# i2Nav-WHU/IC-GVINS

Hardware: NVIDIA H100
Metric: frames/sec (KLT+BA) 1280x560 300-feat 10-KF window (higher is better)
Workload: dtype u8/int32 fixed point + f32 (KLT), f64 (BA)

## Files before the change

### ic_gvins_b200/csrc/ba.cu

```cuda
#include <cooperative_groups.h>
#include <unistd.h>
#include <math.h>
#include <stdlib.h>
#include <string.h>

#include <algorithm>
#include <string>
#include <thread>
#include <vector>

#include "ba_cull.cuh"
#include "ba_slide.cuh"
#include "preint.cuh"
#include "ba_math.cuh"
#include "common.cuh"
#include "geom_core.cuh"

namespace icg {
using namespace bam;
namespace cg = cooperative_groups;

constexpr int BA_SPLIT_W = 4;
constexpr int BA_CHOL_NB = 8;
constexpr int BA_MARG_MAXB = 72;
constexpr int BA_MAX_NODES = 32;

struct BaCaps {
    int NW, K, L, F, G, R;
    int NCV, N, NS, NCA, RJ, LP, NVB;
    int GQ;
};

struct WinDims {
    int K, L, F, n_imu, n_gnss, marg_r, marg_nb;
    int ext_const, td_const, reproj_huber, gnss_huber, has_imu_error, has_pose_prior, has_mix_prior;
    double reproj_sinv;
};

struct LmState {
    double radius, decrease_factor, x_cost, x_norm, cand_cost, model_cost_change, step_norm, gmax, initial_cost;
    double cost_cam[2];
    int iter, n_success, n_invalid, done, need_lin, last_success, first, step_valid, fresh_lin, max_iter, chol_ok;
    int lin_buf;
};

struct ShardDev {
    int split;
    int PK, BS, RV;
    double *peer[8];
    size_t off_inbox, off_bcast, off_scal, off_flagA, off_flagB, off_flagC;
    double *redv;
    int *err;
    double *slm;
    int *slm_cnt;
};

struct BaDev {
    ShardDev S;
    WinDims *dims;
    LmState *st;
    double *pose, *mix, *ext, *rho;
    double *pose_c, *mix_c, *ext_c, *rho_c;
    double *pose_0, *mix_0, *ext_0, *rho_0;
    uint8_t *f_active_0;
    double *gnss_std_0;
    uint8_t *f_active;
    int *lm_off;
    int *lm_perm;
    int *vb_lm0;
    int *ref_nrun;
    int *f_meta_s;
    double *f_const_s;
    int *vis_ord;
    int *part_off, *pair_ro, *npairs;
    double *gpart;
    int *vis_cnt;
    double *Mp[2];
    double *AW[2];
    double *costf[2];
    double *hl[2], *gl[2];
    double *Hc[2], *gc[2];
    double *scale_l, *scale_c;
    double *Hs;
    double *visv;
    double *imu_blob, *imu_U;
    int *gnss_node;
    double *gnss_blh, *gnss_std, *lever;
    double *pose_prior, *pose_prior_sinfo, *mix_prior, *mix_prior_std;
    int *marg_type, *marg_node;
    double *marg_x0, *marg_H0, *marg_b0, *marg_c0;
    double *cost_part;
    double *red2;
    int rank, world;
    double *step_c, *step_l;
    double *Sglobal;
    unsigned long long *clk;
};

__device__ __forceinline__ double *lin_Mp(const BaCaps &C, const BaDev &D, int b, int w) { return D.Mp[b] + (size_t) w * C.K * (C.K - 1) * 210; }
__device__ __forceinline__ double *lin_AW(const BaCaps &C, const BaDev &D, int b, int w) { return D.AW[b] + (size_t) w * C.LP * C.NCA; }
__device__ __forceinline__ double *lin_costf(const BaCaps &C, const BaDev &D, int b, int w) { return D.costf[b] + (size_t) w * C.F; }
__device__ __forceinline__ double *lin_hl(const BaCaps &C, const BaDev &D, int b, int w) { return D.hl[b] + (size_t) w * C.L; }
__device__ __forceinline__ double *lin_gl(const BaCaps &C, const BaDev &D, int b, int w) { return D.gl[b] + (size_t) w * C.L; }
__device__ __forceinline__ double *lin_Hc(const BaCaps &C, const BaDev &D, int b, int w) { return D.Hc[b] + (size_t) w * C.NS * C.NS; }
__device__ __forceinline__ double *lin_gc(const BaCaps &C, const BaDev &D, int b, int w) { return D.gc[b] + (size_t) w * C.NS; }

__device__ __forceinline__ int col_pose(int k) { return 6 * k; }
__device__ __forceinline__ int col_ext(int K) { return 6 * K; }
// ... 670 lines not shown
    __syncthreads();
    if (tid < 9 && dm.has_mix_prior) {
        const double sd = D.mix_prior_std[(size_t) w * 9 + tid];
        Hc[(size_t) (col_mix(K, 0) + tid) * C.NS + col_mix(K, 0) + tid] += 1.0 / (sd * sd);
        gc[col_mix(K, 0) + tid] += s_mp[tid] / sd;
    }
    __syncthreads();
    CAM_CLK(5)
#undef CAM_CLK
    return s_total;
}

constexpr int CAM_THREADS = 320;
__global__ void __launch_bounds__(CAM_THREADS) ba_lin_cam(BaCaps C, BaDev D, int at_cand) {
    extern __shared__ double smem[];
    const int w = blockIdx.x;
    LmState &st = D.st[w];
    if (st.done || !(at_cand ? st.step_valid : st.need_lin)) return;
    if (D.S.split && (w % D.world) != D.rank) return;
    const WinDims dm = D.dims[w];
    const int b = at_cand ? 1 - st.lin_buf : st.lin_buf;
    const double *pose = at_cand ? D.pose_c : D.pose, *mix = at_cand ? D.mix_c : D.mix, *ext = at_cand ? D.ext_c : D.ext;
    double c = cam_factors(C, D, w, dm, pose + (size_t) w * C.K * 7, mix + (size_t) w * C.K * 9, ext + (size_t) w * 8, true, b, smem);
    if (threadIdx.x == 0) st.cost_cam[b] = c;
}

constexpr int SOLVE_THREADS = 256;

__device__ __forceinline__ double block_sum(double v, double *s_red) {
    const int tid = threadIdx.x, lane = tid & 31, warp = tid >> 5;
    for (int o = 16; o > 0; o >>= 1) v += __shfl_down_sync(0xffffffffu, v, o);
    __syncthreads();
    if (lane == 0) s_red[warp] = v;
    __syncthreads();
    double t = 0;
    if (tid == 0) {
        for (int k = 0; k < (int) (blockDim.x >> 5); k++) t += s_red[k];
        s_red[32] = t;
    }
    __syncthreads();
    return s_red[32];
}
__device__ __forceinline__ double block_max(double v, double *s_red) {
    const int tid = threadIdx.x, lane = tid & 31, warp = tid >> 5;
    for (int o = 16; o > 0; o >>= 1) v = fmax(v, __shfl_down_sync(0xffffffffu, v, o));
    __syncthreads();
    if (lane == 0) s_red[warp] = v;
    __syncthreads();
    if (tid == 0) {
        double t = 0;
        for (int k = 0; k < (int) (blockDim.x >> 5); k++) t = fmax(t, s_red[k]);
        s_red[32] = t;
    }
    __syncthreads();
    return s_red[32];
}

__global__ void __launch_bounds__(SOLVE_THREADS, 2) ba_solve(BaCaps C, BaDev D) {
    extern __shared__ double sm[];
    const int w = blockIdx.x, tid = threadIdx.x;
    LmState &st = D.st[w];
    if (st.done) return;
#ifdef ICG_BA_PHASE_CLOCKS
    unsigned long long clk_prev = D.clk ? clock64() : 0ull;
#define SOLVE_CLK(k)                                              \
    if (D.clk && w == 0 && tid == 0) {                            \
        const unsigned long long t_ = clock64();                  \
        atomicAdd(&D.clk[k], t_ - clk_prev), atomicAdd(&D.clk[8 + (k)], 1ull); \
        clk_prev = t_;                                            \
    }
#define SOLVE_CLK_NOW() (D.clk ? clock64() : 0ull)
#define SOLVE_CLK_ADD(k, t0)                                      \
    if (D.clk && w == 0 && tid == 0) atomicAdd(&D.clk[k], clock64() - (t0)), atomicAdd(&D.clk[8 + (k)], 1ull);
#else
#define SOLVE_CLK(k)
#define SOLVE_CLK_NOW() 0ull
#define SOLVE_CLK_ADD(k, t0)
#endif
    const WinDims dm = D.dims[w];
    const int K = dm.K, L = dm.L, NCV = 6 * K + 7, N = 15 * K + 7;
    const int f_first = st.first, f_fresh = st.fresh_lin, f_last = st.last_success, f_iter = st.iter;
    const double f_gmax_old = st.gmax;
    (void) f_gmax_old;
    double *s_red = sm;
    double *s_scale = s_red + 40;
    double *s_g = s_scale + C.NS;
    double *s_rhs = s_g + C.NS;
    double *s_d2 = s_rhs + C.NS;
    double *s_diag = s_d2 + C.NS;
    double *S = s_diag + C.NS;
    const int b = st.lin_buf;
    const double *Hc = lin_Hc(C, D, b, w), *gcam = lin_gc(C, D, b, w), *Hs = D.Hs + (size_t) w * C.NS * C.NS;
    const double *V = D.visv + (size_t) (3 * C.NCV) * w;
    if (tid == 0 && st.need_lin) st.need_lin = 0;
    double *scale_c = D.scale_c + (size_t) w * C.NS;
    const double *hl = lin_hl(C, D, b, w), *gl = lin_gl(C, D, b, w), *scale_l = D.scale_l + (size_t) w * C.L;

    for (int a = tid; a < N; a += SOLVE_THREADS) {
        double g = gcam[a];
        if (a < NCV) g += V[NCV + a];
        s_g[a] = g;
        if (f_first) {
            double h = Hc[(size_t) a * C.NS + a] + (a < NCV ? V[a] : 0.0);
            scale_c[a] = 1.0 / (1.0 + sqrt(h));
        }
    }
    __syncthreads();
    for (int a = tid; a < N; a += SOLVE_THREADS) s_scale[a] = scale_c[a];
    double gmax_now = st.gmax;
    if (f_fresh) {
        double cs = 0, gq = 0;
        const double *costf = lin_costf(C, D, b, w);
        for (int f = tid; f < dm.F; f += SOLVE_THREADS) cs += costf[f];
        for (int l = tid; l < L; l += SOLVE_THREADS) gq = fmax(gq, fabs(gl[l]));
        const double c = block_sum(cs, s_red), gml = block_max(gq, s_red);
        double gm = 0;
        for (int a = tid; a < N; a += SOLVE_THREADS) gm = fmax(gm, fabs(s_g[a]));
        gm = fmax(block_max(gm, s_red), gml);
        gmax_now = gm;
        if (tid == 0) {
            st.x_cost = c + st.cost_cam[b];
            st.gmax = gm;
            if (f_first) st.initial_cost = st.x_cost;
            st.fresh_lin = 0;
        }
        __syncthreads();
    }
    if (f_first) {
        __syncthreads();
        if (tid == 0) st.first = 0;
    }
    {
        int term = 0;
        if (f_iter >= st.max_iter) term = 1;
        else if (f_last && gmax_now <= 1e-10) term = 2;
        else if (f_last && st.radius <= 1e-32) term = 2;
        if (term) {
            __syncthreads();
            if (tid == 0) st.done = term, st.step_valid = 0;
            return;
        }
    }
    __syncthreads();
    if (tid == 0) st.iter++;
    const double radius = st.radius;
    SOLVE_CLK(0)

    constexpr bool async_fill = true;
    if (async_fill) {
        for (int i = tid >> 5; i < N; i += SOLVE_THREADS / 32) {
            const double *src = (i < NCV ? Hs : Hc) + (size_t) i * C.NS;
            const unsigned dst = (unsigned) __cvta_generic_to_shared(S + i * (i + 1) / 2);
            for (int j = tid & 31; j <= i; j += 32)
                asm volatile("cp.async.ca.shared.global [%0], [%1], 8;" ::"r"(dst + 8u * j), "l"(src + j) : "memory");
        }
        asm volatile("cp.async.commit_group;" ::: "memory");
    }
    for (int a = tid; a < N; a += SOLVE_THREADS) {
        double h = Hc[(size_t) a * C.NS + a] + (a < NCV ? V[a] : 0.0);
        double hs = s_scale[a] * s_scale[a] * h;
        s_d2[a] = fmin(fmax(hs, 1e-6), 1e32) / radius;
        double gw = a < NCV ? V[2 * NCV + a] : 0.0;
        s_rhs[a] = -s_scale[a] * (s_g[a] - gw);
    }
    if (async_fill) asm volatile("cp.async.wait_all;" ::: "memory");
    __syncthreads();
    if (async_fill) {
        for (int i = tid >> 5; i < N; i += SOLVE_THREADS / 32) {
            double *row = S + i * (i + 1) / 2;
            const double si = s_scale[i];
            for (int j = tid & 31; j <= i; j += 32) {
                double v = si * s_scale[j] * row[j];
                if (i == j) v += s_d2[i];
                row[j] = v;
            }
        }
    } else {
        for (int i = tid >> 5; i < N; i += SOLVE_THREADS / 32) {
            constexpr int MAXQ = 16;
            double hv[MAXQ];
            const int nq = i / 32 + 1;
#pragma unroll
            for (int q = 0; q < MAXQ; q++) {
                const int j = (tid & 31) + 32 * q;
                hv[q] = 0;
                if (q < nq && j <= i) hv[q] = (i < NCV ? Hs : Hc)[(size_t) i * C.NS + j];
            }
#pragma unroll
            for (int q = 0; q < MAXQ; q++) {
                const int j = (tid & 31) + 32 * q;
                if (q < nq && j <= i) {
                    double v = s_scale[i] * s_scale[j] * hv[q];
                    if (i == j) v += s_d2[i];
                    S[i * (i + 1) / 2 + j] = v;
                }
            }
        }
    }
    for (int a = tid; a < N; a += SOLVE_THREADS) S[N * (N + 1) / 2 + a] = s_rhs[a];
    __syncthreads();
    SOLVE_CLK(1)
    __shared__ int s_fail;
    if (tid == 0) s_fail = 0;
    __syncthreads();
    const int NR = N + 1;
    for (int J0 = 0; J0 < N; J0 += BA_CHOL_NB) {
        const int nb = min(BA_CHOL_NB, N - J0);
        const int lane = tid & 31, warp = tid >> 5, g = lane >> 2, kk = lane & 3;
        const int ntile = (NR - J0 + 7) / 8;
        const unsigned long long pc0 = SOLVE_CLK_NOW();
        (void) pc0;
        const int cb = J0 + g;
        const double *rb = S + (cb < NR ? cb * (cb + 1) / 2 : 0);
        const bool okb = cb < NR;
        if (warp == 0) {
            if (J0 > 0) {
                const double *ra = rb;
                double acc[8] = {0, 0, 0, 0, 0, 0, 0, 0};
                int k0 = 0;
                for (; k0 + 16 <= J0; k0 += 16) {
                    const double x0 = okb ? ra[k0 + kk] : 0.0, x1 = okb ? ra[k0 + 4 + kk] : 0.0, x2 = okb ? ra[k0 + 8 + kk] : 0.0, x3 = okb ? ra[k0 + 12 + kk] : 0.0;
                    dmma884(acc[0], acc[1], x0, x0);
                    dmma884(acc[2], acc[3], x1, x1);
                    dmma884(acc[4], acc[5], x2, x2);
                    dmma884(acc[6], acc[7], x3, x3);
                }
                for (; k0 + 8 <= J0; k0 += 8) {
                    const double x0 = okb ? ra[k0 + kk] : 0.0, x1 = okb ? ra[k0 + 4 + kk] : 0.0;
                    dmma884(acc[0], acc[1], x0, x0);
                    dmma884(acc[2], acc[3], x1, x1);
                }
                const double c0 = (acc[0] + acc[2]) + (acc[4] + acc[6]), c1 = (acc[1] + acc[3]) + (acc[5] + acc[7]);
                const int i = J0 + g;
                if (i < NR) {
                    const int ca = J0 + 2 * kk;
                    if (ca < J0 + nb && ca <= i) S[i * (i + 1) / 2 + ca] -= c0;
                    if (ca + 1 < J0 + nb && ca + 1 <= i) S[i * (i + 1) / 2 + ca + 1] -= c1;
                }
                __syncwarp();
            }
            double Ld[BA_CHOL_NB][BA_CHOL_NB], dinv[BA_CHOL_NB];
            bool bad = false;
#pragma unroll
            for (int a = 0; a < BA_CHOL_NB; a++)
#pragma unroll
                for (int b = 0; b < BA_CHOL_NB; b++) Ld[a][b] = (a < nb && b <= a) ? S[(J0 + a) * (J0 + a + 1) / 2 + J0 + b] : (a == b ? 1.0 : 0.0);
#pragma unroll
            for (int j = 0; j < BA_CHOL_NB; j++) {
                double d = Ld[j][j];
#pragma unroll
                for (int k = 0; k < j; k++) d -= Ld[j][k] * Ld[j][k];
                if (!(d > 0.0) || !isfinite(d)) bad = true;
                const double di = rsqrt(d);
                dinv[j] = di;
                Ld[j][j] = d * di;
#pragma unroll
                for (int a = j + 1; a < BA_CHOL_NB; a++) {
                    double sum = Ld[a][j];
#pragma unroll
                    for (int k = 0; k < j; k++) sum -= Ld[a][k] * Ld[j][k];
                    Ld[a][j] = sum * di;
                }
            }
            __syncwarp();
            if (bad && lane == 0) s_fail = 1;
#pragma unroll
            for (int a2 = 0; a2 < BA_CHOL_NB; a2++) {
                double *ri = S + (J0 + a2) * (J0 + a2 + 1) / 2 + J0;
#pragma unroll
                for (int b = 0; b <= a2; b++)
                    if (lane == ((a2 * 8 + b) & 31) && a2 < nb) ri[b] = Ld[a2][b];
                if (lane == 8 + a2 && a2 < nb) s_diag[J0 + a2] = dinv[a2];
            }
            SOLVE_CLK_ADD(6, pc0)
        } else if (J0 > 0 && warp != 4) {
            constexpr int TPW = 4, NWARP = 6;
            const int wslot = warp < 4 ? warp - 1 : warp - 2;
            for (int t0 = 1 + wslot; t0 < ntile; t0 += TPW * NWARP) {
                const double *ra[TPW];
                bool oka[TPW];
                double acc[TPW][4];
#pragma unroll
                for (int u = 0; u < TPW; u++) {
                    const int ia = J0 + 8 * (t0 + u * NWARP) + g;
                    oka[u] = (t0 + u * NWARP) < ntile && ia < NR;
                    ra[u] = S + (oka[u] ? ia * (ia + 1) / 2 : 0);
                    acc[u][0] = acc[u][1] = acc[u][2] = acc[u][3] = 0;
                }
                for (int k0 = 0; k0 + 8 <= J0; k0 += 8) {
                    const double b0 = okb ? rb[k0 + kk] : 0.0, b1 = okb ? rb[k0 + 4 + kk] : 0.0;
                    double a0[TPW], a1[TPW];
#pragma unroll
                    for (int u = 0; u < TPW; u++) a0[u] = oka[u] ? ra[u][k0 + kk] : 0.0, a1[u] = oka[u] ? ra[u][k0 + 4 + kk] : 0.0;
#pragma unroll
                    for (int u = 0; u < TPW; u++) {
                        dmma884(acc[u][0], acc[u][1], a0[u], b0);
                        dmma884(acc[u][2], acc[u][3], a1[u], b1);
                    }
                }
#pragma unroll
                for (int u = 0; u < TPW; u++) {
                    const double c0 = acc[u][0] + acc[u][2], c1 = acc[u][1] + acc[u][3];
                    const int i = J0 + 8 * (t0 + u * NWARP) + g;
                    if (oka[u]) {
                        const int ca = J0 + 2 * kk;
                        if (ca < J0 + nb && ca <= i) S[i * (i + 1) / 2 + ca] -= c0;
                        if (ca + 1 < J0 + nb && ca + 1 <= i) S[i * (i + 1) / 2 + ca + 1] -= c1;
                    }
                }
            }
        }
        __syncthreads();
        const unsigned long long pc1 = SOLVE_CLK_NOW();
        (void) pc1;
        if (s_fail) break;
        for (int i = J0 + nb + tid; i < NR; i += SOLVE_THREADS) {
            double *ri = S + i * (i + 1) / 2 + J0;
            double x[BA_CHOL_NB];
#pragma unroll
            for (int c = 0; c < BA_CHOL_NB; c++) x[c] = c < nb ? ri[c] : 0.0;
#pragma unroll
            for (int c = 0; c < BA_CHOL_NB; c++) {
                if (c < nb) {
                    const double *lc = S + (J0 + c) * (J0 + c + 1) / 2 + J0;
                    double sum = x[c];
#pragma unroll
                    for (int k = 0; k < c; k++) sum -= x[k] * lc[k];
                    x[c] = sum * s_diag[J0 + c];
                }
            }
#pragma unroll
            for (int c = 0; c < BA_CHOL_NB; c++)
                if (c < nb) ri[c] = x[c];
        }
        __syncthreads();
        SOLVE_CLK_ADD(7, pc1)
    }
    __syncthreads();
    bool valid = !s_fail;
    SOLVE_CLK(2)
    if (valid) {
        double *y = S + N * (N + 1) / 2;
        const int lane = tid & 31;
        for (int J0 = ((N - 1) / BA_CHOL_NB) * BA_CHOL_NB; J0 >= 0; J0 -= BA_CHOL_NB) {
            const int nb = min(BA_CHOL_NB, N - J0);
            if (tid < 32) {
                double x[BA_CHOL_NB];
#pragma unroll
                for (int c = BA_CHOL_NB - 1; c >= 0; c--) {
                    x[c] = 0.0;
                    if (c < nb) {
                        double sum = y[J0 + c];
#pragma unroll
                        for (int k = BA_CHOL_NB - 1; k > c; k--)
                            if (k < nb) sum -= S[(J0 + k) * (J0 + k + 1) / 2 + J0 + c] * x[k];
                        x[c] = sum * s_diag[J0 + c];
                    }
                }
#pragma unroll
                for (int c = 0; c < BA_CHOL_NB; c++)
                    if (c == lane && c < nb) s_rhs[J0 + c] = x[c];
            }
            __syncthreads();
            for (int i = tid; i < J0; i += SOLVE_THREADS) {
                double acc = y[i];
#pragma unroll
                for (int c = BA_CHOL_NB - 1; c >= 0; c--)
                    if (c < nb) acc -= S[(J0 + c) * (J0 + c + 1) / 2 + i] * s_rhs[J0 + c];
                y[i] = acc;
            }
            __syncthreads();
        }
    }
    __syncthreads();
    SOLVE_CLK(3)
    double *step_l = D.step_l + (size_t) w * C.L;
    const double *AW = lin_AW(C, D, b, w);
    double part = 0;
    bool finite = true;
    double *R2 = D.red2 + (size_t) w * 4;
    if (!valid) {
        if (tid == 0) {
            st.chol_ok = 0, st.step_valid = 0;
            R2[0] = 0, R2[1] = 0, R2[2] = 1;
        }
        return;
    }
    for (int a = tid; a < N; a += SOLVE_THREADS) {
        double sp = s_rhs[a];
        finite = finite && isfinite(sp);
        part += -0.5 * sp * (s_scale[a] * s_g[a]) + 0.5 * s_d2[a] * sp * sp;
    }
    double *s_sx = s_diag;
    __syncthreads();
    for (int a = tid; a < NCV; a += SOLVE_THREADS) s_sx[a] = s_scale[a] * s_rhs[a];
    __syncthreads();
    {
        const int lane = tid & 31, warp = tid >> 5;
        constexpr int LB = 8;
        const int lu = ((lane >> 4) & 1) * 4 + ((lane >> 3) & 1) * 2 + ((lane >> 2) & 1);
        for (int l0 = LB * warp; l0 < L; l0 += LB * (SOLVE_THREADS / 32)) {
            const int l = l0 + lu;
            const bool lok = l < L;
            const double sl = lok ? scale_l[l] : 0.0, hh = lok ? hl[l] : 0.0, gg = lok ? gl[l] : 0.0;
            double d[LB];
#pragma unroll
            for (int u = 0; u < LB; u++) d[u] = 0;
            for (int c = lane; c < NCV; c += 32) {
                const double sx = s_sx[c];
#pragma unroll
                for (int u = 0; u < LB; u++) d[u] += (l0 + u < L ? AW[(size_t) (l0 + u) * C.NCA + c] : 0.0) * sx;
            }
            const double hs = sl * sl * hh, d2 = fmin(fmax(hs, 1e-6), 1e32) / radius, den = hs + d2, sg = sl * gg;
            double e4[4], e2[2];
            {
                const bool hi = lane & 16;
#pragma unroll
                for (int u = 0; u < 4; u++) {
                    const double keep = hi ? d[u + 4] : d[u], send = hi ? d[u] : d[u + 4];
                    e4[u] = keep + __shfl_xor_sync(0xffffffffu, send, 16);
                }
            }
            {
                const bool hi = lane & 8;
#pragma unroll
                for (int u = 0; u < 2; u++) {
                    const double keep = hi ? e4[u + 2] : e4[u], send = hi ? e4[u] : e4[u + 2];
                    e2[u] = keep + __shfl_xor_sync(0xffffffffu, send, 8);
                }
            }
            double mine;
            {
                const bool hi = lane & 4;
                const double keep = hi ? e2[1] : e2[0], send = hi ? e2[0] : e2[1];
                mine = keep + __shfl_xor_sync(0xffffffffu, send, 4);
            }
            mine += __shfl_xor_sync(0xffffffffu, mine, 2);
            mine += __shfl_xor_sync(0xffffffffu, mine, 1);
            if ((lane & 3) == 0 && lok) {
                double sp = (-sg - sl * mine) / den;
                finite = finite && isfinite(sp);
                step_l[l] = sp;
                part += -0.5 * sp * sg + 0.5 * d2 * sp * sp;
            }
        }
    }
    __syncthreads();
    SOLVE_CLK(4)
    const double mcc = block_sum(part, s_red);
    const double nfin = block_sum(finite ? 0.0 : 1.0, s_red);
    const double *pose = D.pose + (size_t) w * C.K * 7, *mix = D.mix + (size_t) w * C.K * 9, *ext = D.ext + (size_t) w * 8, *rho = D.rho + (size_t) w * C.L;
    double *pose_c = D.pose_c + (size_t) w * C.K * 7, *mix_c = D.mix_c + (size_t) w * C.K * 9, *ext_c = D.ext_c + (size_t) w * 8, *rho_c = D.rho_c + (size_t) w * C.L;
// ... 463 lines not shown
        return rc_init;
    }
    *out = h;
    return ICG_OK;
}

static int ba_create_body(icg_ba *h, int max_windows, int max_K, int max_L, int max_F, int max_gnss, int max_marg_r, void *stream) {
    if (stream) {
        h->stream = (cudaStream_t) stream;
    } else {
        ICG_CUDA(cudaStreamCreateWithFlags(&h->stream, cudaStreamNonBlocking));
        h->own_stream = true;
    }
    {
        int prio_lo = 0, prio_hi = 0;
        ICG_CUDA(cudaDeviceGetStreamPriorityRange(&prio_lo, &prio_hi));
        ICG_CUDA(cudaStreamCreateWithPriority(&h->stream_cam, cudaStreamNonBlocking, prio_hi));
    }
    ICG_CUDA(cudaEventCreateWithFlags(&h->ev_fork, cudaEventDisableTiming));
    ICG_CUDA(cudaEventCreateWithFlags(&h->ev_join, cudaEventDisableTiming));
    h->prof = getenv("ICG_BA_PROFILE") != nullptr;
    if (h->prof) {
        double *ck = nullptr;
        if (dmalloc(h, &ck, 48) != ICG_OK) return ICG_ENOMEM;
        h->D.clk = (unsigned long long *) ck;
    }
    if (getenv("ICG_BA_PROFILE_SKIP")) h->prof_skip = atoi(getenv("ICG_BA_PROFILE_SKIP"));
    BaCaps &C = h->C;
    max_L = std::max(1, max_L), max_F = std::max(1, max_F);
    C.NW = max_windows, C.K = max_K, C.L = max_L, C.F = max_F, C.G = std::max(1, max_gnss), C.R = std::max(1, max_marg_r);
    C.NCV = 6 * max_K + 7, C.N = 15 * max_K + 7, C.NS = (C.N + 3) & ~3, C.NCA = 4 * ((C.NCV + 1 + 3) / 4);
    C.RJ = (2 * max_F + 31) & ~31, C.LP = (max_L + 31) & ~31;
    C.NVB = (max_F + 127 - max_K) / (128 - max_K) + max_L / 128 + 4 + max_K;
    C.GQ = std::max(1, std::min(max_F, (C.NVB - 2) * (max_K - 1)));
    h->nblk_vis = (max_F + 255) / 256;
    const size_t NW = max_windows;
#define HD(field, count)                                                       \
    if (h->field.alloc(count) != ICG_OK) {                                     \
        set_error("icg_ba_create: allocation of " #field " failed");           \
        return ICG_ENOMEM;                                                     \
    }
    HD(dims, NW) HD(st, NW) HD(pose, NW * C.K * 7) HD(mix, NW * C.K * 9) HD(ext, NW * 8) HD(rho, NW * C.L)
    HD(imu_blob, NW * C.K * ICG_IMU_BLOB_DOUBLES) HD(imu_U, NW * C.K * 225) HD(gnss_blh, NW * C.G * 3) HD(gnss_std, NW * C.G * 3) HD(lever, NW * 3)
    HD(pose_prior, NW * 7) HD(pose_prior_sinfo, NW * 6) HD(mix_prior, NW * 9) HD(mix_prior_std, NW * 9) HD(marg_x0, NW * BA_MARG_MAXB * 9)
    HD(marg_H0, NW * C.R * C.R) HD(marg_b0, NW * C.R) HD(marg_c0, NW)
    HD(lm_off, NW * (C.L + 1)) HD(lm_perm, NW * C.L) HD(lm_fidx, NW * C.F) HD(gnss_node, NW * C.G) HD(marg_type, NW * BA_MARG_MAXB) HD(marg_node, NW * BA_MARG_MAXB) HD(f_active, NW * C.F)
    HD(scratch, 1024) HD(st_save, NW) HD(cull_counters, 2 * NW) HD(f_meta_s, NW * C.F * 4) HD(vb_lm0, NW * C.NVB) HD(ref_nrun, NW * C.K) HD(f_const_s, NW * C.F * 14)
    HD(part_off, NW * ((size_t) C.K * (C.K - 1) + 1)) HD(pair_ro, NW * (size_t) C.K * (C.K - 1)) HD(vis_ord, NW * C.F) HD(npairs, NW)
#undef HD
    ICG_CUDA(cudaMemsetAsync(h->st.d, 0, sizeof(LmState) * NW, h->stream));
    BaDev &D = h->D;
    D.rank = 0, D.world = 1;
    D.dims = h->dims.d, D.st = h->st.d, D.pose = h->pose.d, D.mix = h->mix.d, D.ext = h->ext.d, D.rho = h->rho.d;
    D.f_active = h->f_active.d;
    D.part_off = h->part_off.d, D.pair_ro = h->pair_ro.d, D.vis_ord = h->vis_ord.d, D.npairs = h->npairs.d;
    D.f_meta_s = h->f_meta_s.d, D.vb_lm0 = h->vb_lm0.d, D.ref_nrun = h->ref_nrun.d, D.f_const_s = h->f_const_s.d;
    D.lm_off = h->lm_off.d, D.lm_perm = h->lm_perm.d, D.imu_blob = h->imu_blob.d, D.imu_U = h->imu_U.d;
    D.gnss_node = h->gnss_node.d, D.gnss_blh = h->gnss_blh.d, D.gnss_std = h->gnss_std.d, D.lever = h->lever.d;
    D.pose_prior = h->pose_prior.d, D.pose_prior_sinfo = h->pose_prior_sinfo.d, D.mix_prior = h->mix_prior.d, D.mix_prior_std = h->mix_prior_std.d;
    D.marg_type = h->marg_type.d, D.marg_node = h->marg_node.d, D.marg_x0 = h->marg_x0.d, D.marg_H0 = h->marg_H0.d, D.marg_b0 = h->marg_b0.d, D.marg_c0 = h->marg_c0.d;
    int rc = ICG_OK;
#define DM(field, count) \
    if (rc == ICG_OK) rc = dmalloc(h, &D.field, count);
    DM(pose_c, NW * C.K * 7) DM(mix_c, NW * C.K * 9) DM(ext_c, NW * 8) DM(rho_c, NW * C.L)
    DM(pose_0, NW * C.K * 7) DM(mix_0, NW * C.K * 9) DM(ext_0, NW * 8) DM(rho_0, NW * C.L)
    DM(AW[0], NW * C.NCA * C.LP) DM(Mp[0], NW * (size_t) C.K * (C.K - 1) * 210) DM(visv, NW * 3 * C.NCV)
    DM(gpart, NW * (size_t) C.GQ * 210) DM(costf[0], NW * C.F) DM(hl[0], NW * C.L) DM(gl[0], NW * C.L) DM(scale_l, NW * C.L) DM(scale_c, NW * C.NS)
    DM(Hc[0], NW * C.NS * C.NS) DM(gc[0], NW * C.NS) DM(Hs, NW * C.NS * C.NS) DM(cost_part, NW * (h->nblk_vis + 1)) DM(red2, NW * 4) DM(step_c, NW * C.NS) DM(step_l, NW * C.L)
#undef DM
    if (rc == ICG_OK) rc = dmalloc(h, &D.gnss_std_0, NW * C.G * 3);
    if (rc == ICG_OK) {
        double *cnt = nullptr;
        rc = dmalloc(h, &cnt, (NW * C.K + 1) / 2);
        D.vis_cnt = (int *) cnt;
    }
    if (rc == ICG_OK) {
        double *fa0 = nullptr;
        rc = dmalloc(h, &fa0, (NW * C.F + 7) / 8 + 1);
        D.f_active_0 = (uint8_t *) fa0;
    }
    if (rc != ICG_OK) return rc;
    h->smem_cam = sizeof(double) * ((size_t) C.K * 480 + (size_t) C.G * 24 + 48 + 16 + 2 * (size_t) C.R + 8) + sizeof(int) * (size_t) C.R + 64;
    size_t vec = sizeof(double) * (40 + 5 * (size_t) C.NS);
    size_t packed = sizeof(double) * ((size_t) (C.N + 1) * (C.N + 2) / 2);
    h->use_global_S = (vec + packed > 220 * 1024) ? 1 : 0;
    h->smem_solve = vec + (h->use_global_S ? 0 : packed);
    D.Sglobal = nullptr;
    memset(&D.S, 0, sizeof(D.S));
    if (h->use_global_S) {
        rc = split_setup(h, 0, 1);
        if (rc != ICG_OK) return rc;
    } else {
        ICG_CUDA(raise_dynamic_smem((const void *) ba_solve, (size_t) (h->smem_solve)));
    }
    h->ld_schur = 16 * ((C.NCA + 15) / 16) + 8;
    h->smem_schur = sizeof(double) * std::max((size_t) SCHUR_RCH * h->ld_schur + SCHUR_RCH, (size_t) SCHUR_PASS * 256);
    ICG_CUDA(raise_dynamic_smem((const void *) ba_schur_dmma, (size_t) (h->smem_schur)));
    ICG_CUDA(cudaFuncSetAttribute(ba_schur_dmma, cudaFuncAttributePreferredSharedMemoryCarveout, cudaSharedmemCarveoutMaxShared));
    ICG_CUDA(raise_dynamic_smem((const void *) ba_lin_cam, (size_t) (h->smem_cam)));
    ICG_CUDA(raise_dynamic_smem((const void *) ba_cost_cam, (size_t) (h->smem_cam)));
    ICG_CUDA(raise_dynamic_smem((const void *) ba_lin_vis, LV_SMEM));
    ICG_CUDA(cudaStreamSynchronize(h->stream));
    h->cur_windows = 0;
    return ICG_OK;
}

void icg_ba_destroy(icg_ba *h) {
    if (!h) return;
    cudaSetDevice(h->device);
    if (h->stream) cudaStreamSynchronize(h->stream);
    prof_collect(h);
    prof_print(h);
    for (cudaEvent_t e : h->prof_ev) cudaEventDestroy(e);
    h->dims.release(), h->st.release(), h->pose.release(), h->mix.release(), h->ext.release(), h->rho.release();
    h->imu_blob.release(), h->imu_U.release(), h->gnss_blh.release(), h->gnss_std.release(), h->lever.release(), h->pose_prior.release();
    h->pose_prior_sinfo.release(), h->mix_prior.release(), h->mix_prior_std.release(), h->marg_x0.release(), h->marg_H0.release(), h->marg_b0.release();
    h->marg_c0.release(), h->lm_off.release(), h->lm_perm.release(), h->lm_fidx.release(), h->gnss_node.release();
    h->f_meta_s.release(), h->vb_lm0.release(), h->ref_nrun.release(), h->f_const_s.release(), h->marg_type.release(), h->marg_node.release(), h->f_active.release(), h->scratch.release(), h->st_save.release(), h->cull_counters.release(), h->part_off.release(), h->pair_ro.release(), h->vis_ord.release(), h->npairs.release();
    split_release(h);
    if (h->marg_ready) h->marg_map.release(), h->marg_oJ0.release(), h->marg_oe0.release(), h->marg_oHp.release(), h->marg_obp.release(), h->marg_fmask.release();
    for (double *p : {h->M.H0, h->M.b0, h->M.G1, h->M.V1, h->M.lam1, h->M.Z})
        if (p) cudaFree(p);
    if (h->cull_h) cudaFreeHost(h->cull_h);
    if (h->cull_d) cudaFree(h->cull_d);
    if (h->reint_h) cudaFreeHost(h->reint_h);
    if (h->reint_d) cudaFree(h->reint_d);
    if (h->slide_h) cudaFreeHost(h->slide_h);
    if (h->slide_d) cudaFree(h->slide_d);
    if (h->slide_old) cudaFree(h->slide_old);
    if (h->fc_alt) cudaFree(h->fc_alt);
    if (h->slide_ev) cudaEventDestroy(h->slide_ev);
    for (void *p : h->dev_only) cudaFree(p);
    if (h->stream_cam) cudaStreamSynchronize(h->stream_cam), cudaStreamDestroy(h->stream_cam);
    if (h->ev_fork) cudaEventDestroy(h->ev_fork);
    if (h->ev_join) cudaEventDestroy(h->ev_join);
    if (h->own_stream && h->stream) cudaStreamDestroy(h->stream);
    delete h;
}

#define PK_FAIL(code, ...)                          \
    do {                                            \
        char eb_[512];                              \
        snprintf(eb_, sizeof(eb_), __VA_ARGS__);    \
        err = eb_;                                  \
        return code;                                \
    } while (0)
static int pack_window(icg_ba *h, int w, const icg_ba_problem &p, bool values, std::string &err) {
        const BaCaps &C = h->C;
        if (p.K < 2 || p.K > C.K || p.L < 0 || p.L > C.L || p.F < 0 || p.F > C.F || p.n_imu < 0 || p.n_imu > p.K - 1 || p.n_gnss < 0 || p.n_gnss > C.G ||
            p.marg_r < 0 || p.marg_r > C.R || p.marg_nblocks < 0 || p.marg_nblocks > 2 * C.K + 2 || !p.pose || !p.mix || !p.ext || (p.L > 0 && !p.invdepth) ||
            (p.F > 0 && (!p.f_lm || !p.f_ref || !p.f_obs || !p.f_const))) {
            PK_FAIL(ICG_EINVAL, "icg_ba_upload: window %d exceeds the handle's capacity or has null parameter arrays (K=%d L=%d F=%d gnss=%d marg_r=%d)", w, p.K, p.L, p.F,
                      p.n_gnss, p.marg_r);
        }
        WinDims &d = h->dims.h[w];
        d.K = p.K, d.L = p.L, d.F = p.F, d.n_imu = p.n_imu, d.n_gnss = p.n_gnss, d.marg_r = p.marg_r, d.marg_nb = p.marg_nblocks;
        d.ext_const = p.ext_const != 0, d.td_const = p.td_const != 0, d.reproj_huber = p.reproj_huber != 0, d.gnss_huber = p.gnss_huber != 0;
        d.has_imu_error = p.has_imu_error != 0, d.has_pose_prior = p.has_pose_prior != 0, d.has_mix_prior = p.has_mix_prior != 0;
        d.reproj_sinv = 1.0 / p.reproj_std;
        if (values) {
            memcpy(h->pose.h + (size_t) w * C.K * 7, p.pose, sizeof(double) * 7 * p.K);
            memcpy(h->mix.h + (size_t) w * C.K * 9, p.mix, sizeof(double) * 9 * p.K);
        }
        memcpy(h->ext.h + (size_t) w * 8, p.ext, sizeof(double) * 8);
        if (values && p.L > 0) memcpy(h->rho.h + (size_t) w * C.L, p.invdepth, sizeof(double) * p.L);
        for (int f = 0; f < p.F; f++) {
            if (p.f_lm[f] < 0 || p.f_lm[f] >= p.L || p.f_ref[f] < 0 || p.f_ref[f] >= p.K || p.f_obs[f] < 0 || p.f_obs[f] >= p.K || p.f_ref[f] == p.f_obs[f]) {
                PK_FAIL(ICG_EINVAL, "icg_ba_upload: window %d factor %d has invalid indices", w, f);
            }
// ... 1896 lines not shown
```

Before: 24650.

## Store Cholesky matrix in swizzled 8x8 tiles for vectorized DMMA loads

Replaces the packed lower-triangular row layout of the reduced camera matrix in shared memory with a tiled layout of 8x8 blocks, each swizzled so fragment loads are double2-vectorized and avoid bank conflicts. The fill replaces cp.async row copies with batched __ldcg gathers into tiles, and the RHS is stored as the last tile row. The back-substitution is also restructured so that warp 0 applies the update for the next panel and solves it while the other warps update the remaining entries, removing one barrier per panel. The cost is more shared memory from padded tiles, more complex indexing, and the loss of async copy overlap during the fill.

```diff
diff --git a/ic_gvins_b200/csrc/ba.cu b/ic_gvins_b200/csrc/ba.cu
--- a/ic_gvins_b200/csrc/ba.cu
+++ b/ic_gvins_b200/csrc/ba.cu
@@ -24,6 +24,11 @@
 constexpr int BA_CHOL_NB = 8;
 constexpr int BA_MARG_MAXB = 72;
 constexpr int BA_MAX_NODES = 32;
+
+__host__ __device__ __forceinline__ int st_ntiles(int rows) { return ((rows + 7) >> 3) * (((rows + 7) >> 3) + 1) / 2; }
+__device__ __forceinline__ int st_tile(int T, int c) { return 64 * (T * (T + 1) / 2 + c); }
+__device__ __forceinline__ int st_in(int r, int q) { return 8 * r + 2 * (((q & 3) + (r >> 1)) & 3) + (q >> 2); }
+__device__ __forceinline__ int st_pos(int i, int j) { return st_tile(i >> 3, j >> 3) + st_in(i & 7, j & 7); }
 
 struct BaCaps {
     int NW, K, L, F, G, R;
@@ -860,13 +865,13 @@
     const int f_first = st.first, f_fresh = st.fresh_lin, f_last = st.last_success, f_iter = st.iter;
     const double f_gmax_old = st.gmax;
     (void) f_gmax_old;
-    double *s_red = sm;
+    double *S = sm;
+    double *s_red = S + 64 * st_ntiles(C.N + 1);
     double *s_scale = s_red + 40;
     double *s_g = s_scale + C.NS;
     double *s_rhs = s_g + C.NS;
     double *s_d2 = s_rhs + C.NS;
     double *s_diag = s_d2 + C.NS;
-    double *S = s_diag + C.NS;
     const int b = st.lin_buf;
     const double *Hc = lin_Hc(C, D, b, w), *gcam = lin_gc(C, D, b, w), *Hs = D.Hs + (size_t) w * C.NS * C.NS;
     const double *V = D.visv + (size_t) (3 * C.NCV) * w;
@@ -924,16 +929,6 @@
     const double radius = st.radius;
     SOLVE_CLK(0)
 
-    constexpr bool async_fill = true;
-    if (async_fill) {
-        for (int i = tid >> 5; i < N; i += SOLVE_THREADS / 32) {
-            const double *src = (i < NCV ? Hs : Hc) + (size_t) i * C.NS;
-            const unsigned dst = (unsigned) __cvta_generic_to_shared(S + i * (i + 1) / 2);
-            for (int j = tid & 31; j <= i; j += 32)
-                asm volatile("cp.async.ca.shared.global [%0], [%1], 8;" ::"r"(dst + 8u * j), "l"(src + j) : "memory");
-        }
-        asm volatile("cp.async.commit_group;" ::: "memory");
-    }
     for (int a = tid; a < N; a += SOLVE_THREADS) {
         double h = Hc[(size_t) a * C.NS + a] + (a < NCV ? V[a] : 0.0);
         double hs = s_scale[a] * s_scale[a] * h;
@@ -941,79 +936,83 @@
         double gw = a < NCV ? V[2 * NCV + a] : 0.0;
         s_rhs[a] = -s_scale[a] * (s_g[a] - gw);
     }
-    if (async_fill) asm volatile("cp.async.wait_all;" ::: "memory");
     __syncthreads();
-    if (async_fill) {
-        for (int i = tid >> 5; i < N; i += SOLVE_THREADS / 32) {
-            double *row = S + i * (i + 1) / 2;
-            const double si = s_scale[i];
-            for (int j = tid & 31; j <= i; j += 32) {
-                double v = si * s_scale[j] * row[j];
-                if (i == j) v += s_d2[i];
-                row[j] = v;
-            }
-        }
-    } else {
-        for (int i = tid >> 5; i < N; i += SOLVE_THREADS / 32) {
-            constexpr int MAXQ = 16;
-            double hv[MAXQ];
-            const int nq = i / 32 + 1;
-#pragma unroll
-            for (int q = 0; q < MAXQ; q++) {
-                const int j = (tid & 31) + 32 * q;
-                hv[q] = 0;
-                if (q < nq && j <= i) hv[q] = (i < NCV ? Hs : Hc)[(size_t) i * C.NS + j];
-            }
-#pragma unroll
-            for (int q = 0; q < MAXQ; q++) {
-                const int j = (tid & 31) + 32 * q;
-                if (q < nq && j <= i) {
-                    double v = s_scale[i] * s_scale[j] * hv[q];
-                    if (i == j) v += s_d2[i];
-                    S[i * (i + 1) / 2 + j] = v;
+    const int NR = N + 1, nt = (NR + 7) >> 3, ntl = st_ntiles(NR);
+    {
+        constexpr int TB = 8, NW = SOLVE_THREADS / 32;
+        const int lane = tid & 31;
+        int T = 0, c = tid >> 5;
+        while (c > T) c -= T + 1, T++;
+        for (int t0 = tid >> 5; t0 < ntl; t0 += TB * NW) {
+            int Tb[TB], cb[TB];
+#pragma unroll
+            for (int u = 0; u < TB; u++) {
+                Tb[u] = T, cb[u] = c;
+                c += NW;
+                while (c > T) c -= T + 1, T++;
+            }
+            double v[TB][2];
+#pragma unroll
+            for (int u = 0; u < TB; u++)
+#pragma unroll
+                for (int h = 0; h < 2; h++) {
+                    const int p = lane + 32 * h, r = p >> 3;
+                    const int i = 8 * Tb[u] + r, j = 8 * cb[u] + ((((p >> 1) & 3) - (r >> 1)) & 3) + 4 * (p & 1);
+                    v[u][h] = (t0 + NW * u < ntl && j <= i && i < N) ? __ldcg((i < NCV ? Hs : Hc) + (size_t) i * C.NS + j) : 0.0;
                 }
-            }
-        }
-    }
-    for (int a = tid; a < N; a += SOLVE_THREADS) S[N * (N + 1) / 2 + a] = s_rhs[a];
+#pragma unroll
+            for (int u = 0; u < TB; u++) {
+                const int t = t0 + NW * u;
+#pragma unroll
+                for (int h = 0; h < 2; h++) {
+                    const int p = lane + 32 * h, r = p >> 3;
+                    const int i = 8 * Tb[u] + r, j = 8 * cb[u] + ((((p >> 1) & 3) - (r >> 1)) & 3) + 4 * (p & 1);
+                    double x = 0.0;
+                    if (j <= i && i < N) {
+                        x = s_scale[i] * s_scale[j] * v[u][h];
+                        if (i == j) x += s_d2[i];
+                    } else if (i == N && j < N) {
+                        x = s_rhs[j];
+                    }
+                    if (t < ntl) S[64 * t + p] = x;
+                }
+            }
+        }
+    }
     __syncthreads();
     SOLVE_CLK(1)
     __shared__ int s_fail;
     if (tid == 0) s_fail = 0;
     __syncthreads();
-    const int NR = N + 1;
-    for (int J0 = 0; J0 < N; J0 += BA_CHOL_NB) {
+    for (int J = 0, J0 = 0; J0 < N; J++, J0 += BA_CHOL_NB) {
         const int nb = min(BA_CHOL_NB, N - J0);
         const int lane = tid & 31, warp = tid >> 5, g = lane >> 2, kk = lane & 3;
-        const int ntile = (NR - J0 + 7) / 8;
         const unsigned long long pc0 = SOLVE_CLK_NOW();
         (void) pc0;
-        const int cb = J0 + g;
-        const double *rb = S + (cb < NR ? cb * (cb + 1) / 2 : 0);
-        const bool okb = cb < NR;
+        const double *rb = S + st_tile(J, 0) + st_in(g, kk);
+        double *dg = S + st_tile(J, J);
         if (warp == 0) {
-            if (J0 > 0) {
-                const double *ra = rb;
+            if (J > 0) {
                 double acc[8] = {0, 0, 0, 0, 0, 0, 0, 0};
-                int k0 = 0;
-                for (; k0 + 16 <= J0; k0 += 16) {
-                    const double x0 = okb ? ra[k0 + kk] : 0.0, x1 = okb ? ra[k0 + 4 + kk] : 0.0, x2 = okb ? ra[k0 + 8 + kk] : 0.0, x3 = okb ? ra[k0 + 12 + kk] : 0.0;
-                    dmma884(acc[0], acc[1], x0, x0);
-                    dmma884(acc[2], acc[3], x1, x1);
-                    dmma884(acc[4], acc[5], x2, x2);
-                    dmma884(acc[6], acc[7], x3, x3);
+                int kt = 0;
+                for (; kt + 2 <= J; kt += 2) {
+                    const double2 x01 = *(const double2 *) (rb + 64 * kt), x23 = *(const double2 *) (rb + 64 * (kt + 1));
+                    dmma884(acc[0], acc[1], x01.x, x01.x);
+                    dmma884(acc[2], acc[3], x01.y, x01.y);
+                    dmma884(acc[4], acc[5], x23.x, x23.x);
+                    dmma884(acc[6], acc[7], x23.y, x23.y);
                 }
-                for (; k0 + 8 <= J0; k0 += 8) {
-                    const double x0 = okb ? ra[k0 + kk] : 0.0, x1 = okb ? ra[k0 + 4 + kk] : 0.0;
-                    dmma884(acc[0], acc[1], x0, x0);
-                    dmma884(acc[2], acc[3], x1, x1);
+                for (; kt < J; kt++) {
+                    const double2 x01 = *(const double2 *) (rb + 64 * kt);
+                    dmma884(acc[0], acc[1], x01.x, x01.x);
+                    dmma884(acc[2], acc[3], x01.y, x01.y);
                 }
                 const double c0 = (acc[0] + acc[2]) + (acc[4] + acc[6]), c1 = (acc[1] + acc[3]) + (acc[5] + acc[7]);
                 const int i = J0 + g;
                 if (i < NR) {
-                    const int ca = J0 + 2 * kk;
-                    if (ca < J0 + nb && ca <= i) S[i * (i + 1) / 2 + ca] -= c0;
-                    if (ca + 1 < J0 + nb && ca + 1 <= i) S[i * (i + 1) / 2 + ca + 1] -= c1;
+                    const int ca = 2 * kk;
+                    if (ca < nb && J0 + ca <= i) dg[st_in(g, ca)] -= c0;
+                    if (ca + 1 < nb && J0 + ca + 1 <= i) dg[st_in(g, ca + 1)] -= c1;
                 }
                 __syncwarp();
             }
@@ -1022,7 +1021,7 @@
 #pragma unroll
             for (int a = 0; a < BA_CHOL_NB; a++)
 #pragma unroll
-                for (int b = 0; b < BA_CHOL_NB; b++) Ld[a][b] = (a < nb && b <= a) ? S[(J0 + a) * (J0 + a + 1) / 2 + J0 + b] : (a == b ? 1.0 : 0.0);
+                for (int b = 0; b < BA_CHOL_NB; b++) Ld[a][b] = (a < nb && b <= a) ? dg[st_in(a, b)] : (a == b ? 1.0 : 0.0);
 #pragma unroll
             for (int j = 0; j < BA_CHOL_NB; j++) {
                 double d = Ld[j][j];
@@ -1044,46 +1043,45 @@
             if (bad && lane == 0) s_fail = 1;
 #pragma unroll
             for (int a2 = 0; a2 < BA_CHOL_NB; a2++) {
-                double *ri = S + (J0 + a2) * (J0 + a2 + 1) / 2 + J0;
 #pragma unroll
                 for (int b = 0; b <= a2; b++)
-                    if (lane == ((a2 * 8 + b) & 31) && a2 < nb) ri[b] = Ld[a2][b];
+                    if (lane == ((a2 * 8 + b) & 31) && a2 < nb) dg[st_in(a2, b)] = Ld[a2][b];
                 if (lane == 8 + a2 && a2 < nb) s_diag[J0 + a2] = dinv[a2];
             }
             SOLVE_CLK_ADD(6, pc0)
-        } else if (J0 > 0 && warp != 4) {
+        } else if (J > 0 && warp != 4) {
             constexpr int TPW = 4, NWARP = 6;
             const int wslot = warp < 4 ? warp - 1 : warp - 2;
-            for (int t0 = 1 + wslot; t0 < ntile; t0 += TPW * NWARP) {
-                const double *ra[TPW];
+            for (int T0 = J + 1 + wslot; T0 < nt; T0 += TPW * NWARP) {
+                int ra[TPW];
                 bool oka[TPW];
                 double acc[TPW][4];
 #pragma unroll
                 for (int u = 0; u < TPW; u++) {
-                    const int ia = J0 + 8 * (t0 + u * NWARP) + g;
-                    oka[u] = (t0 + u * NWARP) < ntile && ia < NR;
-                    ra[u] = S + (oka[u] ? ia * (ia + 1) / 2 : 0);
+                    const int T = T0 + u * NWARP;
+                    oka[u] = T < nt && 8 * T + g < NR;
+                    ra[u] = (T < nt ? st_tile(T, 0) : 0) + st_in(g, kk);
                     acc[u][0] = acc[u][1] = acc[u][2] = acc[u][3] = 0;
                 }
-                for (int k0 = 0; k0 + 8 <= J0; k0 += 8) {
-                    const double b0 = okb ? rb[k0 + kk] : 0.0, b1 = okb ? rb[k0 + 4 + kk] : 0.0;
-                    double a0[TPW], a1[TPW];
-#pragma unroll
-                    for (int u = 0; u < TPW; u++) a0[u] = oka[u] ? ra[u][k0 + kk] : 0.0, a1[u] = oka[u] ? ra[u][k0 + 4 + kk] : 0.0;
+                for (int kt = 0; kt < J; kt++) {
+                    const double2 bq = *(const double2 *) (rb + 64 * kt);
+                    double2 aq[TPW];
+#pragma unroll
+                    for (int u = 0; u < TPW; u++) aq[u] = oka[u] ? *(const double2 *) (S + ra[u] + 64 * kt) : make_double2(0.0, 0.0);
 #pragma unroll
                     for (int u = 0; u < TPW; u++) {
-                        dmma884(acc[u][0], acc[u][1], a0[u], b0);
-                        dmma884(acc[u][2], acc[u][3], a1[u], b1);
+                        dmma884(acc[u][0], acc[u][1], aq[u].x, bq.x);
+                        dmma884(acc[u][2], acc[u][3], aq[u].y, bq.y);
                     }
                 }
 #pragma unroll
                 for (int u = 0; u < TPW; u++) {
                     const double c0 = acc[u][0] + acc[u][2], c1 = acc[u][1] + acc[u][3];
-                    const int i = J0 + 8 * (t0 + u * NWARP) + g;
                     if (oka[u]) {
-                        const int ca = J0 + 2 * kk;
-                        if (ca < J0 + nb && ca <= i) S[i * (i + 1) / 2 + ca] -= c0;
-                        if (ca + 1 < J0 + nb && ca + 1 <= i) S[i * (i + 1) / 2 + ca + 1] -= c1;
+                        double *tc = S + st_tile(T0 + u * NWARP, J);
+                        const int ca = 2 * kk;
+                        if (ca < nb) tc[st_in(g, ca)] -= c0;
+                        if (ca + 1 < nb) tc[st_in(g, ca + 1)] -= c1;
                     }
                 }
             }
@@ -1093,23 +1091,25 @@
         (void) pc1;
         if (s_fail) break;
         for (int i = J0 + nb + tid; i < NR; i += SOLVE_THREADS) {
-            double *ri = S + i * (i + 1) / 2 + J0;
+            double *ri = S + st_tile(i >> 3, J) + 8 * (i & 7);
+            const int sh = (i >> 1) & 3;
             double x[BA_CHOL_NB];
 #pragma unroll
-            for (int c = 0; c < BA_CHOL_NB; c++) x[c] = c < nb ? ri[c] : 0.0;
+            for (int m = 0; m < 4; m++) {
+                const double2 p = *(const double2 *) (ri + 2 * ((m + sh) & 3));
+                x[m] = p.x, x[m + 4] = p.y;
+            }
 #pragma unroll
             for (int c = 0; c < BA_CHOL_NB; c++) {
                 if (c < nb) {
-                    const double *lc = S + (J0 + c) * (J0 + c + 1) / 2 + J0;
                     double sum = x[c];
 #pragma unroll
-                    for (int k = 0; k < c; k++) sum -= x[k] * lc[k];
+                    for (int k = 0; k < c; k++) sum -= x[k] * dg[st_in(c, k)];
                     x[c] = sum * s_diag[J0 + c];
                 }
             }
 #pragma unroll
-            for (int c = 0; c < BA_CHOL_NB; c++)
-                if (c < nb) ri[c] = x[c];
+            for (int m = 0; m < 4; m++) *(double2 *) (ri + 2 * ((m + sh) & 3)) = make_double2(x[m], x[m + 4]);
         }
         __syncthreads();
         SOLVE_CLK_ADD(7, pc1)
@@ -1118,34 +1118,50 @@
     bool valid = !s_fail;
     SOLVE_CLK(2)
     if (valid) {
-        double *y = S + N * (N + 1) / 2;
         const int lane = tid & 31;
-        for (int J0 = ((N - 1) / BA_CHOL_NB) * BA_CHOL_NB; J0 >= 0; J0 -= BA_CHOL_NB) {
-            const int nb = min(BA_CHOL_NB, N - J0);
+        for (int a = tid; a < N; a += SOLVE_THREADS) s_rhs[a] = S[st_pos(N, a)];
+        __syncthreads();
+        auto solve_panel = [&](int J) {
+            const int J0 = J * BA_CHOL_NB, nb = min(BA_CHOL_NB, N - J0);
+            const double *dg = S + st_tile(J, J);
+            double x[BA_CHOL_NB];
+#pragma unroll
+            for (int c = BA_CHOL_NB - 1; c >= 0; c--) {
+                x[c] = 0.0;
+                if (c < nb) {
+                    double sum = s_rhs[J0 + c];
+#pragma unroll
+                    for (int k = BA_CHOL_NB - 1; k > c; k--)
+                        if (k < nb) sum -= dg[st_in(k, c)] * x[k];
+                    x[c] = sum * s_diag[J0 + c];
+                }
+            }
+            __syncwarp();
+#pragma unroll
+            for (int c = 0; c < BA_CHOL_NB; c++)
+                if (c == lane && c < nb) s_rhs[J0 + c] = x[c];
+        };
+        auto apply_panel = [&](int J, int i) {
+            const int J0 = J * BA_CHOL_NB, nb = min(BA_CHOL_NB, N - J0);
+            const double *lt = S + st_tile(J, i >> 3);
+            const int q = i & 7;
+            double acc = s_rhs[i];
+#pragma unroll
+            for (int c = BA_CHOL_NB - 1; c >= 0; c--)
+                if (c < nb) acc -= lt[st_in(c, q)] * s_rhs[J0 + c];
+            s_rhs[i] = acc;
+        };
+        const int npan = (N + BA_CHOL_NB - 1) / BA_CHOL_NB;
+        if (tid < 32) solve_panel(npan - 1);
+        __syncthreads();
+        for (int J = npan - 1; J > 0; J--) {
+            const int J0 = J * BA_CHOL_NB;
             if (tid < 32) {
-                double x[BA_CHOL_NB];
-#pragma unroll
-                for (int c = BA_CHOL_NB - 1; c >= 0; c--) {
-                    x[c] = 0.0;
-                    if (c < nb) {
-                        double sum = y[J0 + c];
-#pragma unroll
-                        for (int k = BA_CHOL_NB - 1; k > c; k--)
-                            if (k < nb) sum -= S[(J0 + k) * (J0 + k + 1) / 2 + J0 + c] * x[k];
-                        x[c] = sum * s_diag[J0 + c];
-                    }
-                }
-#pragma unroll
-                for (int c = 0; c < BA_CHOL_NB; c++)
-                    if (c == lane && c < nb) s_rhs[J0 + c] = x[c];
-            }
-            __syncthreads();
-            for (int i = tid; i < J0; i += SOLVE_THREADS) {
-                double acc = y[i];
-#pragma unroll
-                for (int c = BA_CHOL_NB - 1; c >= 0; c--)
-                    if (c < nb) acc -= S[(J0 + c) * (J0 + c + 1) / 2 + i] * s_rhs[J0 + c];
-                y[i] = acc;
+                if (lane < BA_CHOL_NB) apply_panel(J, J0 - BA_CHOL_NB + lane);
+                __syncwarp();
+                solve_panel(J - 1);
+            } else {
+                for (int i = tid - 32; i < J0 - BA_CHOL_NB; i += SOLVE_THREADS - 32) apply_panel(J, i);
             }
             __syncthreads();
         }
@@ -1775,9 +1791,9 @@
     if (rc != ICG_OK) return rc;
     h->smem_cam = sizeof(double) * ((size_t) C.K * 480 + (size_t) C.G * 24 + 48 + 16 + 2 * (size_t) C.R + 8) + sizeof(int) * (size_t) C.R + 64;
     size_t vec = sizeof(double) * (40 + 5 * (size_t) C.NS);
-    size_t packed = sizeof(double) * ((size_t) (C.N + 1) * (C.N + 2) / 2);
-    h->use_global_S = (vec + packed > 220 * 1024) ? 1 : 0;
-    h->smem_solve = vec + (h->use_global_S ? 0 : packed);
+    size_t tiles = sizeof(double) * 64 * (size_t) st_ntiles(C.N + 1);
+    h->use_global_S = (vec + tiles > 220 * 1024) ? 1 : 0;
+    h->smem_solve = vec + (h->use_global_S ? 0 : tiles);
     D.Sglobal = nullptr;
     memset(&D.S, 0, sizeof(D.S));
     if (h->use_global_S) {
```

New measurement: 25440, median of 6. +3.2%, better.
